# study-game-engines/directx-renderer-kurth

Hardware: AMD Instinct MI355X
Metric: physics steps/sec at 100k rigid bodies (higher is better)
Workload: dtype f32; 1 GPU; c3: 100k mixed colliders (sphere/capsule/OBB), dt 1/120 s, 30 solver iterations; bodies=100000, broadphase_pairs=611032, manifolds=251275, contacts=317267, joints=0, recoveries=0, parallelism=1 gpu

## Files before the change

### directx-renderer-kurth_amd/csrc/k_cluster_solve.hip

```cpp
#include "cluster.h"
#include "solver_rows.h"
#include "joint_solve.h"

#define CL_MAX_LOCAL_TASKS 8u
#define CLS_LANES 512u
#define CLQ_QUADS (CLS_LANES / 4u)
#define CLQ_SETS 7u
#define CLQ_REG_CONTACTS (CLQ_QUADS * CLQ_SETS)
#define CLQ_SETS_JOINTS 4u
#define CL_SPIN_LIMIT (1u << 22)

typedef u32 u32x4 __attribute__((ext_vector_type(4)));

struct QuadRow { V3 dT, aT, dN, aN; float mT, mN, bias, friction, lamN, lamT; };
#define CLQ_ZERO_FLOAT4S (2u * CLQ_QUADS + 4u)
#define CLQ_ROW_FLOAT4S 14u

struct ClLocal
{
	u32 first, count, numBodies, numShared, numColors, serialStart, numContacts, phase, key, sharedBase, numJoints;
	u32 bodyOff;
	u32 infoOff;
	u32 regContacts;
	u32 rowOff;
	u32 rowCap;
	u32 scratchBase;
	u32 colorStart[68];
};

struct ClArgs
{
	u32* counters; const ClTask* tasks; const u32* bodyList; const u32* phaseMask; const u32* sharedSlot;
	const u32* mKeySorted; const u32* mLocal; const u32* cEntry;
	const float4* rowPlanes; const float4* rowShared; float2* rowLambda; float4* rowScratch; u32 scratchContacts;
	u32 regContactsCap;
	u32 predictDiv, pollSleep;
	float4* vel; u64* flow; u64* trace;
	size_t rowCap; u32 nb, flowBytes, epoch, itBegin, itEnd, ldsFloat4s;
	const u32* jointClassStart; const uint2* taskJoints; const uint4* jointTable; float* jointUpd[MI_JOINT_TYPES]; const float4* invIw; u32 numJointClasses;
};

MI_DEV float clQuadSum(float p)
{
	float q = p + __builtin_bit_cast(float, __builtin_amdgcn_update_dpp(0, __builtin_bit_cast(int, p), 0xB1, 0xF, 0xF, false));
	return q + __builtin_bit_cast(float, __builtin_amdgcn_update_dpp(0, __builtin_bit_cast(int, q), 0x4E, 0xF, 0xF, false));
}
MI_DEV void clSolveQuad(QuadRow& r, V3& x)
{
	float vt = clQuadSum(rowDot3(x, r.dT));
	float maxFriction = r.friction * r.lamN;
	float newT = rowClampSym(__builtin_fmaf(-r.mT, vt, r.lamT), maxFriction);
	float d = newT - r.lamT; r.lamT = newT;
	x = rowFma(d, r.aT, x);
	float vn = clQuadSum(rowDot3(x, r.dN));
	float newN = fmaxf(__builtin_fmaf(-r.mN, vn - r.bias, r.lamN), 0.f);
	d = newN - r.lamN; r.lamN = newN;
	x = rowFma(d, r.aN, x);
}
// ... 18 lines not shown
template <typename PTR> MI_DEV void clStoreQuadRow(PTR P, u32 q, const QuadRow& r, u32 addr)
{
	P[3u * q] = make_float4(r.dT.x, r.dT.y, r.dT.z, r.aT.x); P[3u * q + 1u] = make_float4(r.aT.y, r.aT.z, r.dN.x, r.dN.y); P[3u * q + 2u] = make_float4(r.dN.z, r.aN.x, r.aN.y, r.aN.z);
	if (q == 0u) P[12] = make_float4(r.mT, r.mN, r.bias, r.friction);
	const u32 other = (u32)__builtin_amdgcn_update_dpp(0, (int)addr, 0xB1, 0xF, 0xF, false);
	const u32 otherPair = (u32)__builtin_amdgcn_update_dpp(0, (int)(addr | (other << 16)), 0x4E, 0xF, 0xF, false);
	if (q == 0u) P[13] = make_float4(r.lamN, r.lamT, __uint_as_float(addr | (other << 16)), __uint_as_float(otherPair));
}
MI_DEV u32 clPairAddr(u32 pair, u32 q) { return (q & 1u) ? (pair >> 16) : (pair & 0xFFFFu); }
#define CLQ_PAIR_WORD(q) (54u + ((q) >> 1))
template <typename PTR> MI_DEV void clLoadQuadRow(QuadRow& r, u32& addr, PTR P, u32 q)
{
	float4 a = P[3u * q], b = P[3u * q + 1u], c = P[3u * q + 2u], d = P[12], e = P[13];
	r.dT = v3f4(a); r.aT = v3(a.w, b.x, b.y); r.dN = v3(b.z, b.w, c.x); r.aN = v3(c.y, c.z, c.w);
	r.mT = d.x; r.mN = d.y; r.bias = d.z; r.friction = d.w; r.lamN = e.x; r.lamT = e.y;
	addr = clPairAddr(__float_as_uint(q < 2u ? e.z : e.w), q);
}

template <bool JOINTS> __global__ void __launch_bounds__(CLS_LANES) k_cl_solve(ClArgs A)
{
	extern __shared__ float4 lds[];
	__shared__ ClLocal sTask[CL_MAX_LOCAL_TASKS];
	__shared__ u32 sNumTasks, sAbort;
	const u32 tid = threadIdx.x, G = gridDim.x, quad = tid >> 2, q = tid & 3u;
	constexpr u32 SETS = JOINTS ? CLQ_SETS_JOINTS : CLQ_SETS;
	u32* status = A.counters + CTR_FLOW_STATUS;
	__amdgpu_buffer_rsrc_t rsrc = __builtin_amdgcn_make_buffer_rsrc(A.flow, 0, A.flowBytes, 0x00020000);
	const u32 zeroBase = A.ldsFloat4s - CLQ_ZERO_FLOAT4S, zeroRec = zeroBase + 2u * CLQ_QUADS, sinkRec = zeroRec + 2u;

	if (tid == 0)
	{
		if (A.trace) A.trace[(size_t)blockIdx.x * CL_TRACE_ROWS * CL_TRACE_WORDS + 15 * 32] = wall_clock64();
		u32 nT = 0, off = 0, used = 0;
		bool bad = A.counters[CTR_CL_STATUS] != 0u;
		for (u32 p = 0; p < CL_MAX_PHASES; ++p)
		{
			u32 tasksInPhase = A.counters[CTR_CL_NUM_TASKS + p];
			if (tasksInPhase > CL_TASKS_PER_PHASE * G) { bad = true; atomicOr(status, 128u); }
			off = clPhaseOffset(A.counters, p);
			u32 t = (blockIdx.x + G - (off % G)) % G;
			for (; t < tasksInPhase && !bad; t += G)
			{
				u32 key = p * CL_MAX_TASKS + t;
				const ClTask* T = A.tasks + key;
				const u32 tj = (A.jointClassStart && p == 0u) ? A.jointClassStart[(size_t)key * (CL_MAX_JOINT_CLASSES + 2u) + CL_MAX_JOINT_CLASSES] : 0u;
				if (!T->count && !tj) continue;
				if (nT == CL_MAX_LOCAL_TASKS) { bad = true; atomicOr(status, 256u); break; }
				ClLocal& L = sTask[nT];
				L.first = T->first; L.count = T->count; L.numBodies = T->numBodies; L.numShared = T->numShared; L.numColors = T->numColors; L.serialStart = T->serialStart; L.numContacts = T->numRows;
				L.phase = p; L.key = key; L.sharedBase = T->sharedBase; L.numJoints = tj;
				if (tj > CLS_LANES || (tj && nT)) { bad = true; atomicOr(status, 2048u); }
				for (u32 c = 0; c <= CL_SERIAL_COLOR + 1u; ++c) L.colorStart[c] = T->colorStart[c];
				L.colorStart[CL_SERIAL_COLOR + 2u] = L.colorStart[CL_SERIAL_COLOR + 1u]; L.colorStart[CL_SERIAL_COLOR + 3u] = L.colorStart[CL_SERIAL_COLOR + 1u];
				L.bodyOff = used; used += 2u * L.numBodies;
				L.infoOff = used * 4u; used += (3u * L.numBodies + 3u) / 4u;
				L.regContacts = (nT == 0) ? min(L.numContacts, min(CLQ_QUADS * SETS, A.regContactsCap)) : 0u;
				L.rowOff = 0; L.rowCap = 0;
				++nT;
			}
		}
		if (used + CLQ_ZERO_FLOAT4S > A.ldsFloat4s) { bad = true; atomicOr(status, 512u); }
		for (u32 k = 0; k < nT && !bad; ++k)
		{
			ClLocal& L = sTask[k];
			u32 want = L.numContacts - L.regContacts;
			u32 left = A.ldsFloat4s - used - CLQ_ZERO_FLOAT4S;
			u32 fit = left / CLQ_ROW_FLOAT4S;
			u32 cap = want < fit ? want : fit;
			L.rowOff = used; L.rowCap = cap; used += CLQ_ROW_FLOAT4S * cap; L.scratchBase = 0;
			if (want > cap) { L.scratchBase = atomicAdd(&A.counters[CTR_CL_SCRATCH], want - cap); if (L.scratchBase + (want - cap) > A.scratchContacts) { bad = true; atomicOr(status, 1024u); break; } }
		}
		if (bad) atomicOr(status, 64u);
		sNumTasks = nT; sAbort = (bad || __hip_atomic_load(status, __ATOMIC_RELAXED, __HIP_MEMORY_SCOPE_AGENT) != 0u) ? 1u : 0u;
	}
	__syncthreads();
	if (sAbort) return;
	const u32 numTasks = sNumTasks;
	if (!numTasks) return;

	for (u32 k = 0; k < numTasks; ++k)
	{
		const ClLocal& L = sTask[k];
		u32* info = (u32*)lds + L.infoOff;
		for (u32 l = tid; l < L.numBodies; l += CLS_LANES)
		{
			u32 g = A.bodyList[(size_t)L.key * CL_BODY_STRIDE + l];
			u32 pm = A.phaseMask[g];
			u32 deg = __popc(pm), rank = __popc(pm & ((1u << L.phase) - 1u));
			u32 below = pm & ((1u << L.phase) - 1u);
			u32 prev = below ? 31u - (u32)__clz(below) : 31u - (u32)__clz(pm);
			info[3 * l] = g; info[3 * l + 1] = deg | (rank << 8);
			info[3 * l + 2] = (l < L.numShared) ? A.sharedSlot[(size_t)prev * (A.nb + 1u) + g] : 0u;
			lds[L.bodyOff + 2 * l] = A.vel[2 * g]; lds[L.bodyOff + 2 * l + 1] = A.vel[2 * g + 1];
		}
	}
	for (u32 i = tid; i < CLQ_ZERO_FLOAT4S; i += CLS_LANES) lds[zeroBase + i] = make_float4(0.f, 0.f, 0.f, 0.f);
	__syncthreads();
	QuadRow rows[SETS]; u32 addr[SETS];
	{
		const ClLocal& L = sTask[0];
#pragma unroll
		for (u32 s = 0; s < SETS; ++s)
		{
			const u32 p = s * CLQ_QUADS + quad;
			rows[s].dT = rows[s].aT = rows[s].dN = rows[s].aN = v3(0.f, 0.f, 0.f); rows[s].mT = rows[s].mN = rows[s].bias = rows[s].friction = rows[s].lamN = rows[s].lamT = 0.f; addr[s] = sinkRec;
			if (p < L.regContacts) { u32 slot, kk; clBuildQuadRow(rows[s], addr[s], L, A, lds, p, q, zeroBase + 2u * quad, slot, kk); }
		}
	}
	for (u32 k = 0; k < numTasks; ++k)
	{
		const ClLocal& L = sTask[k];
		for (u32 i = quad; i < L.numContacts - L.regContacts; i += CLQ_QUADS)
		{
			QuadRow r; u32 a, slot, kk;
			clBuildQuadRow(r, a, L, A, lds, L.regContacts + i, q, zeroBase + 2u * quad, slot, kk);
			if (i < L.rowCap) clStoreQuadRow(lds + L.rowOff + i * CLQ_ROW_FLOAT4S, q, r, a);
			else clStoreQuadRow(A.rowScratch + (size_t)(L.scratchBase + i - L.rowCap) * CLQ_ROW_FLOAT4S, q, r, a);
		}
	}
	u32 tailStart0 = sTask[0].numColors, tailSet = 0, myTail = 255u;
	{
		const ClLocal& L = sTask[0];
		const u32 endPos = L.colorStart[L.numColors];
		if (L.numColors && endPos && endPos <= L.regContacts)
		{
			const u32 blk = (endPos - 1u) >> 4;
			while (tailStart0 > 0u && (L.colorStart[tailStart0 - 1u] >> 4) == blk) --tailStart0;
			if (L.numColors - tailStart0 < 2u) tailStart0 = L.numColors;
			else
			{
				tailSet = L.colorStart[tailStart0] / CLQ_QUADS;
				const u32 p = tailSet * CLQ_QUADS + quad;
				if (p >= L.colorStart[tailStart0] && p < endPos) { myTail = tailStart0; while (L.colorStart[myTail + 1u] <= p) ++myTail; }
			}
		}
		tailStart0 = __builtin_amdgcn_readfirstlane(tailStart0); tailSet = __builtin_amdgcn_readfirstlane(tailSet);
	}
	const u32 bodyOff0 = sTask[0].bodyOff;
	u32 jClass = 0xFFFFFFFFu, jType = 0, jA = 0, jB = 0, jRdA = zeroRec, jWrA = sinkRec, jRdB = zeroRec, jWrB = sinkRec; float* jRec = nullptr;
	const u32 numJoints0 = (JOINTS && sTask[0].phase == 0u) ? sTask[0].numJoints : 0u;
	if (JOINTS && tid < numJoints0)
	{
		const u32* cs = A.jointClassStart + (size_t)sTask[0].key * (CL_MAX_JOINT_CLASSES + 2u);
		uint2 e = A.taskJoints[cs[CL_MAX_JOINT_CLASSES + 1u] + tid];
		uint4 t4 = A.jointTable[e.x];
		jType = t4.x & 0xFFu; jClass = t4.x >> 8; jA = t4.z; jB = t4.w;
		jRec = A.jointUpd[jType] + (size_t)t4.y * jointUpdateFloats(jType);
		u32 la = e.y & 0xFFFFu, lb = e.y >> 16;
		if (la != CL_LOCAL_STATIC) { jRdA = bodyOff0 + 2u * la; jWrA = jRdA; }
		if (lb != CL_LOCAL_STATIC) { jRdB = bodyOff0 + 2u * lb; jWrB = jRdB; }
	}
	__syncthreads();
	u64* trace = A.trace ? A.trace + (size_t)blockIdx.x * CL_TRACE_ROWS * CL_TRACE_WORDS : nullptr;
	if (trace && tid == 0)
	{
		trace[15 * 32 + 1] = wall_clock64();
		for (u32 k = 0; k < numTasks && k < 5u; ++k) { trace[15 * 32 + 2 + 4 * k] = sTask[k].count; trace[15 * 32 + 3 + 4 * k] = sTask[k].numColors; trace[15 * 32 + 4 + 4 * k] = sTask[k].numShared; trace[15 * 32 + 5 + 4 * k] = sTask[k].phase | (sTask[k].numBodies << 8) | ((u64)sTask[k].numContacts << 32); trace[15 * 32 + 22 + k] = sTask[k].rowCap | ((u64)sTask[k].regContacts << 32); }
	}

#define CLQ_SOLVE_SET(S_, CS_, END_) if ((S_) < SETS) { const u32 pos = (S_) * CLQ_QUADS + quad; if (pos >= (CS_) && pos < (END_)) { float4 b = lds[addr[(S_) < SETS ? (S_) : 0u]]; V3 x = v3f4(b); clSolveQuad(rows[(S_) < SETS ? (S_) : 0u], x); lds[addr[(S_) < SETS ? (S_) : 0u]] = make_float4(x.x, x.y, x.z, b.w); } }
#define CLQ_PREFETCH(POS_) { const u32 in_ = max((POS_), regC) + quad - regC; if (in_ < rowCap) pfW = ((const u32*)(lds + rowOff + in_ * CLQ_ROW_FLOAT4S))[CLQ_PAIR_WORD(q)]; }
#define CLQ_SOLVE_ROWS(CS_, END_) \
	{ \
		u32 w = pfW; \
		CLQ_PREFETCH(END_) \
		for (u32 p = max((CS_), regC) + quad; p < (END_); p += CLQ_QUADS) \
		{ \
			const u32 i = p - regC; \
			QuadRow r; u32 a; float4 b; \
			float4* P = lds + rowOff + i * CLQ_ROW_FLOAT4S; \
			float4* S = A.rowScratch + (size_t)(scratchBase + i - rowCap) * CLQ_ROW_FLOAT4S; \
			u32 wn = 0u; if (p + CLQ_QUADS < (END_) && i + CLQ_QUADS < rowCap) wn = ((const u32*)(P + CLQ_QUADS * CLQ_ROW_FLOAT4S))[CLQ_PAIR_WORD(q)]; \
			if (i < rowCap) { u32 unused; a = clPairAddr(w, q); b = lds[a]; clLoadQuadRow(r, unused, P, q); } else { clLoadQuadRow(r, a, S, q); b = lds[a]; } \
			V3 x = v3f4(b); clSolveQuad(r, x); lds[a] = make_float4(x.x, x.y, x.z, b.w); \
			if (q == 0u) { if (i < rowCap) ((float2*)(P + 13))[0] = make_float2(r.lamN, r.lamT); else ((float2*)(S + 13))[0] = make_float2(r.lamN, r.lamT); } \
			w = wn; \
		} \
	}
#define CLQ_SOLVE_ROWS_LDS(CS_, END_) \
	{ \
		const u32 i = (CS_) - regC + quad, endR = (END_) - regC, w = pfW; \
		pfW = clLdsAt<u32>(lds, __umul24(min(endR + quad, lastRow), CLQ_ROW_FLOAT4S * 16u) + pairByte); \
		if (i < endR) \
		{ \
			const u32 a = clPairAddr(w, q), rowByte = __umul24(i, CLQ_ROW_FLOAT4S * 16u) + rowsByte, own = rowByte + q * 48u; \
			const float4 b = lds[a], r0 = clLdsAt<float4>(lds, own), r1 = clLdsAt<float4>(lds, own + 16u), r2 = clLdsAt<float4>(lds, own + 32u), r3 = clLdsAt<float4>(lds, rowByte + 192u); \
			const float2 lam = clLdsAt<float2>(lds, rowByte + 208u); \
			QuadRow r; r.dT = v3f4(r0); r.aT = v3(r0.w, r1.x, r1.y); r.dN = v3(r1.z, r1.w, r2.x); r.aN = v3(r2.y, r2.z, r2.w); \
			r.mT = r3.x; r.mN = r3.y; r.bias = r3.z; r.friction = r3.w; r.lamN = lam.x; r.lamT = lam.y; \
			V3 x = v3f4(b); clSolveQuad(r, x); lds[a] = make_float4(x.x, x.y, x.z, b.w); \
			if (q == 0u) *(float2*)((char*)lds + (rowByte + 208u)) = make_float2(r.lamN, r.lamT); \
		} \
	}
#define CLQ_ADVANCE(END_) \
	__syncthreads(); \
	if (stamp && c < 63u && (END_) == csNext) { trace[5 * 32 + 1 + c] = clock64(); trace[7 * 32 + c] = csNext - L.colorStart[c]; } \
	if ((END_) == csNext) { csCur = csNext; csNext = __builtin_amdgcn_readfirstlane(csAfter); ++c; } else csCur = (END_);
#define CLQ_SET_LOOP(S_) \
	if ((S_) < SETS) while (c < mainColors && csCur < min(regC, ((S_) + 1u) * CLQ_QUADS)) \
	{ \
		const u32 csAfter = L.colorStart[c + 2u];  \
		const u32 end = min(csNext, min(regC, ((S_) + 2u) * CLQ_QUADS));  \
		CLQ_SOLVE_SET(S_, csCur, end) \
		if (end > ((S_) + 1u) * CLQ_QUADS) { CLQ_SOLVE_SET((S_) + 1u, csCur, end) } \
		CLQ_ADVANCE(end) \
	}
	static_assert(CLQ_SETS <= 8u, "the colour loop below names eight sets");

	bool aborted = false;
#define CLQ_PREFETCH_TURN(K_) { const ClLocal& N = sTask[K_]; const u32 rc = N.regContacts, in_ = max(N.colorStart[0], rc) + quad - rc; if (in_ < N.rowCap) pfW = ((const u32*)(lds + N.rowOff + in_ * CLQ_ROW_FLOAT4S))[CLQ_PAIR_WORD(q)]; }
	u32 pfW = 0u;
	CLQ_PREFETCH_TURN(0u)
	u64 lastPublish = 0; u32 lastWait = 0;
	for (u32 it = A.itBegin; it < A.itEnd && !aborted; ++it)
	{
		for (u32 k = 0; k < numTasks; ++k)
		{
			const ClLocal& L = sTask[k];
			const u32* info = (const u32*)lds + L.infoOff;
			{
				if (k == 0 && lastWait > 64u && it > A.itBegin + 1u)
				{
					u64 until = lastPublish + (u64)(lastWait - lastWait / A.predictDiv);
					while (wall_clock64() < until) __builtin_amdgcn_s_sleep(8);
				}
				const u32 rel = it - A.itBegin;
				for (u32 base = 0; base < L.numShared; base += 2u * CLS_LANES)
				{
					u32 gid[2], want[2]; bool pend[2]; bool any = false;
#pragma unroll
					for (u32 qq = 0; qq < 2; ++qq)
					{
						u32 l = base + qq * CLS_LANES + tid;
// ... 40 lines not shown
			if (k == 0 && it > A.itBegin) lastWait = (u32)(wall_clock64() - lastPublish);
			if (trace && tid == 0 && it - A.itBegin < 32u && k < 5u) trace[(3 * k) * 32 + (it - A.itBegin)] = wall_clock64();
			if (JOINTS && k == 0 && numJoints0)
			{
				const u32* cs = A.jointClassStart + (size_t)L.key * (CL_MAX_JOINT_CLASSES + 2u);
				for (u32 c = 0; c < A.numJointClasses; ++c)
				{
					if (cs[c + 1u] == cs[c]) continue;
					if (jClass == c)
					{
						Vel v; float4 a0 = lds[jRdA], a1 = lds[jRdA + 1], b0 = lds[jRdB], b1 = lds[jRdB + 1];
						v.vA = v3f4(a0); v.wA = v3f4(a1); v.vB = v3f4(b0); v.wB = v3f4(b1); v.invMassA = a0.w; v.invMassB = b0.w;
						M3 IA = ldInvI(A.invIw, jA), IB = ldInvI(A.invIw, jB);
						jointSolve(jType, jRec, v, IA, IB);
						lds[jWrA] = make_float4(v.vA.x, v.vA.y, v.vA.z, v.invMassA); lds[jWrA + 1] = make_float4(v.wA.x, v.wA.y, v.wA.z, 0.f);
						lds[jWrB] = make_float4(v.vB.x, v.vB.y, v.vB.z, v.invMassB); lds[jWrB + 1] = make_float4(v.wB.x, v.wB.y, v.wB.z, 0.f);
					}
					__syncthreads();
				}
			}
			{
				const u32 numColors = __builtin_amdgcn_readfirstlane(L.numColors), serialStart = __builtin_amdgcn_readfirstlane(L.serialStart), numContacts = __builtin_amdgcn_readfirstlane(L.numContacts);
				const u32 regC = __builtin_amdgcn_readfirstlane(L.regContacts), rowOff = __builtin_amdgcn_readfirstlane(L.rowOff), rowCap = __builtin_amdgcn_readfirstlane(L.rowCap), scratchBase = __builtin_amdgcn_readfirstlane(L.scratchBase);
				const bool stamp = trace && tid == 0 && it == A.itBegin + 10u && k == 0;
				if (stamp) trace[5 * 32] = clock64();
				const u32 mainColors = (k == 0u) ? tailStart0 : numColors;
				u32 c = 0, csCur = __builtin_amdgcn_readfirstlane(L.colorStart[0]), csNext = __builtin_amdgcn_readfirstlane(L.colorStart[1]);
				CLQ_SET_LOOP(0) CLQ_SET_LOOP(1) CLQ_SET_LOOP(2) CLQ_SET_LOOP(3) CLQ_SET_LOOP(4) CLQ_SET_LOOP(5) CLQ_SET_LOOP(6) CLQ_SET_LOOP(7)
				if (rowCap >= numContacts - regC)
				{
					const u32 rowsByte = rowOff * 16u, lastRow = max(numContacts - regC, 1u) - 1u, pairByte = rowsByte + 4u * CLQ_PAIR_WORD(q);
					while (c < mainColors)
					{
						const u32 csAfter = L.colorStart[c + 2u];
						const u32 end = min(csNext, csCur + CLQ_QUADS);
						CLQ_SOLVE_ROWS_LDS(csCur, end)
						CLQ_ADVANCE(end)
					}
				}
				else while (c < mainColors)
				{
					const u32 csAfter = L.colorStart[c + 2u];
					CLQ_SOLVE_ROWS(csCur, csNext)
					CLQ_ADVANCE(csNext)
				}
				if (mainColors < numColors)
				{
#define CLQ_TAIL(S_) case S_: if ((S_) < SETS && myTail != 255u) for (u32 ct = mainColors; ct < numColors; ++ct) { if (myTail == ct) { float4 b = lds[addr[(S_) < SETS ? (S_) : 0u]]; V3 x = v3f4(b); clSolveQuad(rows[(S_) < SETS ? (S_) : 0u], x); lds[addr[(S_) < SETS ? (S_) : 0u]] = make_float4(x.x, x.y, x.z, b.w); } __builtin_amdgcn_fence(__ATOMIC_ACQ_REL, "wavefront"); } break;
					switch (tailSet) { CLQ_TAIL(0) CLQ_TAIL(1) CLQ_TAIL(2) CLQ_TAIL(3) CLQ_TAIL(4) CLQ_TAIL(5) CLQ_TAIL(6) CLQ_TAIL(7) default: break; }
#undef CLQ_TAIL
					__syncthreads();
					if (stamp) for (u32 ct = mainColors; ct < numColors && ct < 63u; ++ct) { trace[5 * 32 + 1 + ct] = clock64(); trace[7 * 32 + ct] = L.colorStart[ct + 1u] - L.colorStart[ct]; }
				}
				if (serialStart < numContacts) CLQ_PREFETCH(serialStart)
				for (u32 sp = serialStart; sp < numContacts; ++sp)
				{
					if (sp < regC)
					{
						switch (sp / CLQ_QUADS)
						{
							case 0: CLQ_SOLVE_SET(0u, sp, sp + 1u) break; case 1: CLQ_SOLVE_SET(1u, sp, sp + 1u) break; case 2: CLQ_SOLVE_SET(2u, sp, sp + 1u) break; case 3: CLQ_SOLVE_SET(3u, sp, sp + 1u) break;
							case 4: CLQ_SOLVE_SET(4u, sp, sp + 1u) break; case 5: CLQ_SOLVE_SET(5u, sp, sp + 1u) break; case 6: CLQ_SOLVE_SET(6u, sp, sp + 1u) break; default: CLQ_SOLVE_SET(7u, sp, sp + 1u) break;
						}
					}
					else { CLQ_SOLVE_ROWS(sp, sp + 1u) }
					__syncthreads();
				}
			}
			if (trace && tid == 0 && it - A.itBegin < 32u && k < 5u) trace[(3 * k + 1) * 32 + (it - A.itBegin)] = wall_clock64();
			for (u32 l = tid; l < L.numShared; l += CLS_LANES)
			{
				u32 g = info[3 * l], ti = info[3 * l + 1];
				u32 deg = ti & 0xFFu, rank = ti >> 8;
				u32 want = A.epoch + (it - A.itBegin) * deg + rank;
				u32 rec = (L.sharedBase + l) * 32u;
				float4 b0 = lds[L.bodyOff + 2 * l], b1 = lds[L.bodyOff + 2 * l + 1];
				if (it + 1u == A.itEnd && rank + 1u == deg) { A.vel[2 * g] = b0; A.vel[2 * g + 1] = make_float4(b1.x, b1.y, b1.z, 0.f); }
				else
				{
					u32x4 h1 = { __float_as_uint(b1.x), __float_as_uint(b1.y), __float_as_uint(b1.z), want + 1u };
					u32x4 h0 = { __float_as_uint(b0.x), __float_as_uint(b0.y), __float_as_uint(b0.z), want + 1u };
					__builtin_amdgcn_raw_buffer_store_b128(h1, rsrc, rec + 16u, 0, 16);
					__builtin_amdgcn_raw_buffer_store_b128(h0, rsrc, rec, 0, 16);
				}
			}
// ... 1 lines not shown
			CLQ_PREFETCH_TURN(k + 1u < numTasks ? k + 1u : 0u)
		}
	}
	if (aborted) return;

	for (u32 k = 0; k < numTasks; ++k)
	{
		const ClLocal& L = sTask[k];
		const u32* info = (const u32*)lds + L.infoOff;
		for (u32 l = L.numShared + tid; l < L.numBodies; l += CLS_LANES)
		{
			u32 g = info[3 * l];
			float4 b1 = lds[L.bodyOff + 2 * l + 1];
			A.vel[2 * g] = lds[L.bodyOff + 2 * l]; A.vel[2 * g + 1] = make_float4(b1.x, b1.y, b1.z, 0.f);
		}
		if (q == 0u)
		{
			if (k == 0)
			{
#pragma unroll
				for (u32 s = 0; s < SETS; ++s)
				{
					const u32 p = s * CLQ_QUADS + quad;
					if (p < L.regContacts) { const u32 e = A.cEntry[(size_t)4u * L.first + p]; A.rowLambda[(size_t)(e >> 12) * A.rowCap + L.first + (e & 0xFFFu)] = make_float2(rows[s].lamN, rows[s].lamT); }
				}
			}
			for (u32 i = quad; i < L.numContacts - L.regContacts; i += CLQ_QUADS)
			{
				const u32 e = A.cEntry[(size_t)4u * L.first + L.regContacts + i];
				const float4 lam = i < L.rowCap ? lds[L.rowOff + i * CLQ_ROW_FLOAT4S + 13u] : A.rowScratch[(size_t)(L.scratchBase + i - L.rowCap) * CLQ_ROW_FLOAT4S + 13u];
				A.rowLambda[(size_t)(e >> 12) * A.rowCap + L.first + (e & 0xFFFu)] = make_float2(lam.x, lam.y);
			}
		}
	}
#undef CLQ_SET_LOOP
#undef CLQ_ADVANCE
#undef CLQ_SOLVE_ROWS
#undef CLQ_SOLVE_ROWS_LDS
#undef CLQ_PREFETCH
#undef CLQ_PREFETCH_TURN
#undef CLQ_SOLVE_SET
}

bool cluster_solves_joints(const World& w) { return w.cluster.jointsInCluster && w.cluster.jointsEnabled; }

u32 cluster_solve_setup(const World& w)
{
	int maxLds = 0;
	MI_CHECK(hipDeviceGetAttribute(&maxLds, hipDeviceAttributeMaxSharedMemoryPerBlock, w.device));
	hipFuncAttributes fa = {};
	MI_CHECK(hipFuncGetAttributes(&fa, (const void*)k_cl_solve<true>));
	size_t dyn = (maxLds > 0 ? (size_t)maxLds : 65536) - fa.sharedSizeBytes - 256;
	dyn &= ~(size_t)15;
// ... 24 lines not shown

void launch_cluster_solve(World& w, u32 itBegin, u32 itEnd)
{
	if (itBegin >= itEnd) return;
	size_t words = (size_t)(w.nb + 1) * CL_MAX_PHASES * 4;
	if (w.cluster.flow.cap < words) { w.cluster.flow.ensure(words, w.stream); w.cluster.flowEpoch = 0; if (w.lastError) return; }
	if (w.cluster.flowEpoch == 0 || w.cluster.flowEpoch >= 0xFFFEu)
	{
		MI_CHECK(hipMemsetAsync(w.cluster.flow.p, 0, sizeof(u64) * words, w.stream));
		w.cluster.flowEpoch = 0;
	}
	w.cluster.flowEpoch++;
	if (w.cluster.flowTestAbortStep == w.stats.numInternalSteps)
	{
		u32 one = 16u;
		MI_CHECK(hipMemcpyAsync(w.dCounters.p + CTR_FLOW_STATUS, &one, sizeof(u32), hipMemcpyHostToDevice, w.stream));
		MI_CHECK(hipStreamSynchronize(w.stream));
	}
	const size_t scratchContacts = std::min<size_t>(2 * w.pairCap, 512u * 1024u);
	w.cluster.rowScratch.ensure(scratchContacts * CLQ_ROW_FLOAT4S, w.stream);
	if (w.lastError) return;
	if (itBegin) MI_CHECK(hipMemsetAsync(w.dCounters.p + CTR_CL_SCRATCH, 0, sizeof(u32), w.stream));
	ClArgs A;
	A.rowScratch = w.cluster.rowScratch.p; A.scratchContacts = (u32)scratchContacts; A.regContactsCap = w.cluster.regContactsCap;
	A.counters = w.dCounters.p; A.tasks = (const ClTask*)w.cluster.tasks.p; A.bodyList = w.cluster.bodyList.p; A.phaseMask = w.cluster.phaseMask.p; A.sharedSlot = w.cluster.sharedSlot.p;
	A.mKeySorted = w.mKeySorted.p; A.mLocal = w.cluster.local.p; A.cEntry = w.cluster.entry.p;
	A.rowPlanes = w.rowPlanes.p; A.rowShared = w.rowShared.p; A.rowLambda = w.rowLambda.p; A.vel = w.vel.p; A.flow = w.cluster.flow.p; A.trace = w.cluster.flowTrace.p; A.predictDiv = CL_PREDICT_DIV; A.pollSleep = CL_POLL_SLEEP;
	A.rowCap = w.rowCap; A.nb = w.nb; A.flowBytes = (u32)(words * sizeof(u64)); A.epoch = w.cluster.flowEpoch << 16; A.itBegin = itBegin; A.itEnd = itEnd;
	A.ldsFloat4s = w.cluster.ldsBytes / 16u;
	const bool withJoints = cluster_solves_joints(w);
	A.jointClassStart = withJoints ? w.cluster.jointClassStart.p : nullptr; A.taskJoints = w.cluster.taskJoints.p; A.jointTable = w.cluster.jointTable.p; A.invIw = w.invIw.p; A.numJointClasses = withJoints ? w.cluster.numJointClasses : 0u;
	for (u32 t = 0; t < MI_JOINT_TYPES; ++t) A.jointUpd[t] = w.joints[t].dUpdate.p;
	if (withJoints) hipLaunchKernelGGL(k_cl_solve<true>, dim3(w.cluster.blocks), dim3(CLS_LANES), w.cluster.ldsBytes, w.stream, A);
	else hipLaunchKernelGGL(k_cl_solve<false>, dim3(w.cluster.blocks), dim3(CLS_LANES), w.cluster.ldsBytes, w.stream, A);
}
```

### directx-renderer-kurth_amd/csrc/world.h

```cpp
#pragma once
#include "mi_common.h"
#include "../../include/mi_physics.h"
#include <vector>
#include <string>
#include <algorithm>
#include <type_traits>

struct mi_distance_constraint { float localAnchorA[3], localAnchorB[3], globalLength; };
struct mi_ball_constraint { float localAnchorA[3], localAnchorB[3]; };
struct mi_fixed_constraint { float initialInvRotationDifference[4], localAnchorA[3], localAnchorB[3]; };
struct mi_hinge_constraint
{
	float localAnchorA[3], localAnchorB[3], localHingeAxisA[3], localHingeAxisB[3];
	float minRotationLimit, maxRotationLimit, maxMotorTorque; u32 motorType; float motorVelocity;
	float localHingeTangentA[3], localHingeBitangentA[3], localHingeTangentB[3];
};
struct mi_cone_twist_constraint
{
	float localAnchorA[3], localAnchorB[3], localLimitAxisA[3], localLimitAxisB[3];
	float localLimitTangentA[3], localLimitBitangentA[3], localLimitTangentB[3];
	float swingLimit, twistLimit; u32 swingMotorType; float swingMotorVelocity, maxSwingMotorTorque, swingMotorAxis;
	u32 twistMotorType; float twistMotorVelocity, maxTwistMotorTorque;
};
struct mi_slider_constraint
// ... 193 lines not shown
	{
		std::vector<HCloth> cloths;
		bool dirty = true, stateOnDevice = false;
		u32 iterations[3] = { 0, 1, 0 };
		DevBuf<float> planes; u32 stride = 0;
		DevBuf<uint2> ab; DevBuf<float2> restIms; DevBuf<float4> temp; DevBuf<uint8_t> descs; DevBuf<u32> list;
		u32 numSmall = 0, maxSmallParticles = 0;
	} cloth;
	void uploadCloths(); void downloadCloths();

	struct Slab
	{
		DevBuf<uint8_t> code; DevBuf<u32> fresh; u32 rank = 0, size = 0, axis = 0, stamp = 0; float lo = 0.f, hi = 0.f, margin = 0.f;
	} slab;

	struct Cluster
	{
		bool enabled = true;
		bool jointsEnabled = true;
		u32 blocksLimit = 0, failStreak = 0, taskWeight = 64u * 1000u, taskWeightLater = 64u * 500u;
		u32 taskWeightComp = 64u * 200u;
		u32 ldsBytes = 0, blocks = 0, cooldown = 0;
		u32 regContactsCap = ~0u;
		bool compIdle = false;

		bool sortDue = true; u32 sortAge = 0, sortBodies = 0;
		DevBuf<u32> keys, keysSorted, vals, sorted, rank, wsum, cum, taskKey, taskPos, taskCount;
		DevBuf<u32> jointBodyMask; bool jointListsValid = false;
		DevBuf<u32> compLabel, leftList;
		DevBuf<u32> chunk; u32 chunkJointVersion = ~0u; bool chunkWithJoints = false;
		DevBuf<u32> rep, jointTask, jointPos, jointCount; u32 numJoints = 0;

		DevBuf<u32> phaseMask, pre, local, entry, taskStart, bodyList, sharedSlot;
		DevBuf<uint8_t> tasks;
		DevBuf<float4> rowScratch;
		DevBuf<u32> jointStart, jointList; DevBuf<uint4> jointTable; DevBuf<uint2> taskJoints; DevBuf<u32> jointClassStart;
		u32 numJointClasses = 0; bool jointsInCluster = false;
		DevBuf<u64> flow;
		DevBuf<u64> flowTrace;
		u32 flowEpoch = 0;
		DevBuf<float4> velBackup; u32 flowTestAbortStep = ~0u;
	} cluster;
	void recoverFlow(); int resolvePendingFlow();

	struct Zones
	{
// ... 106 lines not shown
```

### directx-renderer-kurth_amd/csrc/world.hip

```cpp
#include "world.h"
#include <cstdio>
#include <cstring>
#include <atomic>

thread_local std::string g_createError;
thread_local World* g_currentWorld = nullptr;

void mi_set_error(hipError_t e, const char* file, int line)
{
	char buf[512];
	snprintf(buf, sizeof(buf), "HIP error %d (%s) at %s:%d", (int)e, hipGetErrorString(e), file, line);
	if (g_currentWorld) { if (!g_currentWorld->lastError) { g_currentWorld->lastError = MI_ERR_HIP; g_currentWorld->lastErrorText = buf; } }
	else g_createError = buf;
}

template <typename T> void DevBuf<T>::ensure(size_t n, hipStream_t s, bool keep)
{
	if (n <= cap) return;
	size_t newCap = std::max(n, cap + cap / 2);
	T* np = nullptr;
	MI_CHECK(hipMalloc((void**)&np, newCap * sizeof(T)));
	if (!np) return;
	if (keep && p && cap) { MI_CHECK(hipMemcpyAsync(np, p, cap * sizeof(T), hipMemcpyDeviceToDevice, s)); MI_CHECK(hipStreamSynchronize(s)); }
	if (p) MI_CHECK(hipFree(p));
// ... 11 lines not shown
	if (const char* e = getenv("MI_NARROW_SIDE_STREAM")) narrowSideStream = atoi(e) != 0;
	if (narrowSideStream)
	{
		MI_CHECK(hipStreamCreateWithFlags(&narrowStream, hipStreamNonBlocking));
		MI_CHECK(hipEventCreateWithFlags(&narrowFork, hipEventDisableTiming | hipEventDisableSystemFence));
		MI_CHECK(hipEventCreateWithFlags(&narrowJoin, hipEventDisableTiming | hipEventDisableSystemFence));
		if (!narrowStream || !narrowFork || !narrowJoin) narrowSideStream = false;
	}
	MI_CHECK(hipHostMalloc((void**)&hCounters, CTR_WORDS * sizeof(u32), hipHostMallocDefault));
	if (hCounters) memset(hCounters, 0, CTR_WORDS * sizeof(u32));
	dCounters.ensure(CTR_WORDS, stream);
	if (dCounters.p) MI_CHECK(hipMemsetAsync(dCounters.p, 0, CTR_WORDS * sizeof(u32), stream));
	timing.stageEvents.resize(STAGE_RING * 6);
	for (auto& e : timing.stageEvents) MI_CHECK(hipEventCreateWithFlags(&e, hipEventDisableSystemFence));
	MI_CHECK(hipEventCreateWithFlags(&countersEvent, hipEventDisableTiming));
	validate = getenv("MI_PHYSICS_VALIDATE") != nullptr;
	cluster.enabled = getenv("MI_PHYSICS_NO_CLUSTER") == nullptr;
	cluster.jointsEnabled = getenv("MI_CLUSTER_NO_JOINTS") == nullptr;
	if (const char* e = getenv("MI_FLOW_TEST_ABORT")) cluster.flowTestAbortStep = (u32)atoi(e);
	if (const char* e = getenv("MI_CLUSTER_TASK")) { cluster.taskWeight = 64u * (u32)std::max(16, atoi(e)); cluster.taskWeightLater = std::min(cluster.taskWeight, cluster.taskWeightLater); cluster.taskWeightComp = std::min(cluster.taskWeight, cluster.taskWeightComp); }
	if (getenv("MI_PHYSICS_REPLAY")) replay.referenceOrder = true;
	if (const char* e = getenv("MI_CLUSTER_BLOCKS")) cluster.blocksLimit = (u32)std::max(1, atoi(e));
	if (const char* e = getenv("MI_CLUSTER_REG_CONTACTS")) cluster.regContactsCap = (u32)std::max(0, atoi(e));
	if (const char* e = getenv("MI_CLUSTER_TASK_LATER")) cluster.taskWeightLater = 64u * (u32)std::max(16, atoi(e));
	if (const char* e = getenv("MI_CLUSTER_TASK_COMP")) cluster.taskWeightComp = 64u * (u32)std::min(1 << 20, std::max(16, atoi(e)));
	if (dCounters.p)
	{
		u32 box[6] = { 0xFFFFFFFFu, 0xFFFFFFFFu, 0xFFFFFFFFu, 0u, 0u, 0u };
		MI_CHECK(hipMemcpyAsync(dCounters.p + CTR_CL_BBOX, box, sizeof(box), hipMemcpyHostToDevice, stream));
		MI_CHECK(hipStreamSynchronize(stream));
	}
}

World::~World()
{
	g_currentWorld = this;
	if (narrowStream) (void)hipStreamSynchronize(narrowStream);
	if (stream) (void)hipStreamSynchronize(stream);
	for (auto& e : timing.stageEvents) if (e) (void)hipEventDestroy(e);
	if (countersEvent) (void)hipEventDestroy(countersEvent);
	if (hCounters) (void)hipHostFree(hCounters);
	if (narrowFork) (void)hipEventDestroy(narrowFork);
	if (narrowJoin) (void)hipEventDestroy(narrowJoin);
	if (narrowStream) (void)hipStreamDestroy(narrowStream);
	if (stream) (void)hipStreamDestroy(stream);
	g_currentWorld = nullptr;
// ... 376 lines not shown
```

Measured before the change: 579.1 steps/s.

## Reorder contact placement: spill rows first, LDS rows next, register rows last

Rearranges where each cluster task's contact rows live in the solve order. Rows spilled to global scratch now come first, LDS-resident rows follow, and register-held quads take the tail of the contact range instead of the head. Colour iteration becomes three phases (scratch, LDS fast path, register sets), with register colour starts rebased in a shared array. The aim is to keep the fast LDS-only loop even when some rows spill, and to let the register tail line up with the final colours. It also adds an MI_CLUSTER_LDS_ROWS cap for experiments, at the cost of more complex indexing and new edge cases at colour boundaries.

```diff
diff --git a/directx-renderer-kurth_amd/csrc/k_cluster_solve.hip b/directx-renderer-kurth_amd/csrc/k_cluster_solve.hip
--- a/directx-renderer-kurth_amd/csrc/k_cluster_solve.hip
+++ b/directx-renderer-kurth_amd/csrc/k_cluster_solve.hip
@@ -21,10 +21,8 @@
 	u32 first, count, numBodies, numShared, numColors, serialStart, numContacts, phase, key, sharedBase, numJoints;
 	u32 bodyOff;
 	u32 infoOff;
-	u32 regContacts;
-	u32 rowOff;
-	u32 rowCap;
-	u32 scratchBase;
+	u32 regContacts, spill, rowOff, rowCap, scratchBase;
+	u32 ldsColors;
 	u32 colorStart[68];
 };
 
@@ -34,6 +32,7 @@
 	const u32* mKeySorted; const u32* mLocal; const u32* cEntry;
 	const float4* rowPlanes; const float4* rowShared; float2* rowLambda; float4* rowScratch; u32 scratchContacts;
 	u32 regContactsCap;
+	u32 ldsRowsCap;
 	u32 predictDiv, pollSleep;
 	float4* vel; u64* flow; u64* trace;
 	size_t rowCap; u32 nb, flowBytes, epoch, itBegin, itEnd, ldsFloat4s;
@@ -98,6 +97,7 @@
 	extern __shared__ float4 lds[];
 	__shared__ ClLocal sTask[CL_MAX_LOCAL_TASKS];
 	__shared__ u32 sNumTasks, sAbort;
+	__shared__ u32 sRegStart[CL_SERIAL_COLOR + 4u];
 	const u32 tid = threadIdx.x, G = gridDim.x, quad = tid >> 2, q = tid & 3u;
 	constexpr u32 SETS = JOINTS ? CLQ_SETS_JOINTS : CLQ_SETS;
 	u32* status = A.counters + CTR_FLOW_STATUS;
@@ -131,19 +131,23 @@
 				L.bodyOff = used; used += 2u * L.numBodies;
 				L.infoOff = used * 4u; used += (3u * L.numBodies + 3u) / 4u;
 				L.regContacts = (nT == 0) ? min(L.numContacts, min(CLQ_QUADS * SETS, A.regContactsCap)) : 0u;
-				L.rowOff = 0; L.rowCap = 0;
+				L.rowOff = 0; L.rowCap = 0; L.spill = 0;
+				const u32 regBase = L.numContacts - L.regContacts;
+				L.ldsColors = 0; while (L.ldsColors < L.numColors && L.colorStart[L.ldsColors + 1u] <= regBase) ++L.ldsColors;
+				if (nT == 0) for (u32 c = 0; c < CL_SERIAL_COLOR + 4u; ++c) sRegStart[c] = L.colorStart[c] - regBase;
 				++nT;
 			}
 		}
 		if (used + CLQ_ZERO_FLOAT4S > A.ldsFloat4s) { bad = true; atomicOr(status, 512u); }
+		u32 ldsRowsLeft = A.ldsRowsCap;
 		for (u32 k = 0; k < nT && !bad; ++k)
 		{
 			ClLocal& L = sTask[k];
 			u32 want = L.numContacts - L.regContacts;
 			u32 left = A.ldsFloat4s - used - CLQ_ZERO_FLOAT4S;
-			u32 fit = left / CLQ_ROW_FLOAT4S;
+			u32 fit = min(left / CLQ_ROW_FLOAT4S, ldsRowsLeft);
 			u32 cap = want < fit ? want : fit;
-			L.rowOff = used; L.rowCap = cap; used += CLQ_ROW_FLOAT4S * cap; L.scratchBase = 0;
+			L.rowOff = used; L.rowCap = cap; used += CLQ_ROW_FLOAT4S * cap; ldsRowsLeft -= cap; L.scratchBase = 0; L.spill = want - cap;
 			if (want > cap) { L.scratchBase = atomicAdd(&A.counters[CTR_CL_SCRATCH], want - cap); if (L.scratchBase + (want - cap) > A.scratchContacts) { bad = true; atomicOr(status, 1024u); break; } }
 		}
 		if (bad) atomicOr(status, 64u);
@@ -175,38 +179,39 @@
 	QuadRow rows[SETS]; u32 addr[SETS];
 	{
 		const ClLocal& L = sTask[0];
+		const u32 regBase = L.numContacts - L.regContacts;
 #pragma unroll
 		for (u32 s = 0; s < SETS; ++s)
 		{
 			const u32 p = s * CLQ_QUADS + quad;
 			rows[s].dT = rows[s].aT = rows[s].dN = rows[s].aN = v3(0.f, 0.f, 0.f); rows[s].mT = rows[s].mN = rows[s].bias = rows[s].friction = rows[s].lamN = rows[s].lamT = 0.f; addr[s] = sinkRec;
-			if (p < L.regContacts) { u32 slot, kk; clBuildQuadRow(rows[s], addr[s], L, A, lds, p, q, zeroBase + 2u * quad, slot, kk); }
+			if (p < L.regContacts) { u32 slot, kk; clBuildQuadRow(rows[s], addr[s], L, A, lds, regBase + p, q, zeroBase + 2u * quad, slot, kk); }
 		}
 	}
 	for (u32 k = 0; k < numTasks; ++k)
 	{
 		const ClLocal& L = sTask[k];
-		for (u32 i = quad; i < L.numContacts - L.regContacts; i += CLQ_QUADS)
+		for (u32 p = quad; p < L.numContacts - L.regContacts; p += CLQ_QUADS)
 		{
 			QuadRow r; u32 a, slot, kk;
-			clBuildQuadRow(r, a, L, A, lds, L.regContacts + i, q, zeroBase + 2u * quad, slot, kk);
-			if (i < L.rowCap) clStoreQuadRow(lds + L.rowOff + i * CLQ_ROW_FLOAT4S, q, r, a);
-			else clStoreQuadRow(A.rowScratch + (size_t)(L.scratchBase + i - L.rowCap) * CLQ_ROW_FLOAT4S, q, r, a);
+			clBuildQuadRow(r, a, L, A, lds, p, q, zeroBase + 2u * quad, slot, kk);
+			if (p >= L.spill) clStoreQuadRow(lds + L.rowOff + (p - L.spill) * CLQ_ROW_FLOAT4S, q, r, a);
+			else clStoreQuadRow(A.rowScratch + (size_t)(L.scratchBase + p) * CLQ_ROW_FLOAT4S, q, r, a);
 		}
 	}
 	u32 tailStart0 = sTask[0].numColors, tailSet = 0, myTail = 255u;
 	{
 		const ClLocal& L = sTask[0];
-		const u32 endPos = L.colorStart[L.numColors];
-		if (L.numColors && endPos && endPos <= L.regContacts)
-		{
-			const u32 blk = (endPos - 1u) >> 4;
-			while (tailStart0 > 0u && (L.colorStart[tailStart0 - 1u] >> 4) == blk) --tailStart0;
+		const u32 regBase = L.numContacts - L.regContacts, endPos = L.colorStart[L.numColors];
+		if (L.numColors && endPos > regBase)
+		{
+			const u32 blk = (endPos - regBase - 1u) >> 4;
+			while (tailStart0 > 0u && L.colorStart[tailStart0 - 1u] >= regBase && ((L.colorStart[tailStart0 - 1u] - regBase) >> 4) == blk) --tailStart0;
 			if (L.numColors - tailStart0 < 2u) tailStart0 = L.numColors;
 			else
 			{
-				tailSet = L.colorStart[tailStart0] / CLQ_QUADS;
-				const u32 p = tailSet * CLQ_QUADS + quad;
+				tailSet = (L.colorStart[tailStart0] - regBase) / CLQ_QUADS;
+				const u32 p = regBase + tailSet * CLQ_QUADS + quad;
 				if (p >= L.colorStart[tailStart0] && p < endPos) { myTail = tailStart0; while (L.colorStart[myTail + 1u] <= p) ++myTail; }
 			}
 		}
@@ -231,31 +236,31 @@
 	if (trace && tid == 0)
 	{
 		trace[15 * 32 + 1] = wall_clock64();
-		for (u32 k = 0; k < numTasks && k < 5u; ++k) { trace[15 * 32 + 2 + 4 * k] = sTask[k].count; trace[15 * 32 + 3 + 4 * k] = sTask[k].numColors; trace[15 * 32 + 4 + 4 * k] = sTask[k].numShared; trace[15 * 32 + 5 + 4 * k] = sTask[k].phase | (sTask[k].numBodies << 8) | ((u64)sTask[k].numContacts << 32); trace[15 * 32 + 22 + k] = sTask[k].rowCap | ((u64)sTask[k].regContacts << 32); }
+		for (u32 k = 0; k < numTasks && k < 5u; ++k) { trace[15 * 32 + 2 + 4 * k] = sTask[k].count; trace[15 * 32 + 3 + 4 * k] = sTask[k].numColors; trace[15 * 32 + 4 + 4 * k] = sTask[k].numShared; trace[15 * 32 + 5 + 4 * k] = sTask[k].phase | (sTask[k].numBodies << 8) | ((u64)sTask[k].numContacts << 32); trace[15 * 32 + 22 + k] = sTask[k].rowCap | ((u64)sTask[k].regContacts << 32); trace[15 * 32 + 27 + k] = sTask[k].spill | ((u64)(k == 0u ? sTask[0].numColors - tailStart0 : 0u) << 32); }
 	}
 
 #define CLQ_SOLVE_SET(S_, CS_, END_) if ((S_) < SETS) { const u32 pos = (S_) * CLQ_QUADS + quad; if (pos >= (CS_) && pos < (END_)) { float4 b = lds[addr[(S_) < SETS ? (S_) : 0u]]; V3 x = v3f4(b); clSolveQuad(rows[(S_) < SETS ? (S_) : 0u], x); lds[addr[(S_) < SETS ? (S_) : 0u]] = make_float4(x.x, x.y, x.z, b.w); } }
-#define CLQ_PREFETCH(POS_) { const u32 in_ = max((POS_), regC) + quad - regC; if (in_ < rowCap) pfW = ((const u32*)(lds + rowOff + in_ * CLQ_ROW_FLOAT4S))[CLQ_PAIR_WORD(q)]; }
+#define CLQ_PREFETCH(POS_) { const u32 in_ = max((POS_), spill) + quad - spill; if (in_ < rowCap) pfW = ((const u32*)(lds + rowOff + in_ * CLQ_ROW_FLOAT4S))[CLQ_PAIR_WORD(q)]; }
 #define CLQ_SOLVE_ROWS(CS_, END_) \
 	{ \
 		u32 w = pfW; \
 		CLQ_PREFETCH(END_) \
-		for (u32 p = max((CS_), regC) + quad; p < (END_); p += CLQ_QUADS) \
+		for (u32 p = (CS_) + quad; p < (END_); p += CLQ_QUADS) \
 		{ \
-			const u32 i = p - regC; \
+			const bool inLds = p >= spill; \
 			QuadRow r; u32 a; float4 b; \
-			float4* P = lds + rowOff + i * CLQ_ROW_FLOAT4S; \
-			float4* S = A.rowScratch + (size_t)(scratchBase + i - rowCap) * CLQ_ROW_FLOAT4S; \
-			u32 wn = 0u; if (p + CLQ_QUADS < (END_) && i + CLQ_QUADS < rowCap) wn = ((const u32*)(P + CLQ_QUADS * CLQ_ROW_FLOAT4S))[CLQ_PAIR_WORD(q)]; \
-			if (i < rowCap) { u32 unused; a = clPairAddr(w, q); b = lds[a]; clLoadQuadRow(r, unused, P, q); } else { clLoadQuadRow(r, a, S, q); b = lds[a]; } \
+			float4* P = lds + rowOff + (inLds ? p - spill : 0u) * CLQ_ROW_FLOAT4S; \
+			float4* S = A.rowScratch + (size_t)(scratchBase + (inLds ? 0u : p)) * CLQ_ROW_FLOAT4S; \
+			u32 wn = 0u; if (p + CLQ_QUADS < (END_) && p + CLQ_QUADS >= spill) wn = ((const u32*)(lds + rowOff + (p + CLQ_QUADS - spill) * CLQ_ROW_FLOAT4S))[CLQ_PAIR_WORD(q)]; \
+			if (inLds) { u32 unused; a = clPairAddr(w, q); b = lds[a]; clLoadQuadRow(r, unused, P, q); } else { clLoadQuadRow(r, a, S, q); b = lds[a]; } \
 			V3 x = v3f4(b); clSolveQuad(r, x); lds[a] = make_float4(x.x, x.y, x.z, b.w); \
-			if (q == 0u) { if (i < rowCap) ((float2*)(P + 13))[0] = make_float2(r.lamN, r.lamT); else ((float2*)(S + 13))[0] = make_float2(r.lamN, r.lamT); } \
+			if (q == 0u) { if (inLds) ((float2*)(P + 13))[0] = make_float2(r.lamN, r.lamT); else ((float2*)(S + 13))[0] = make_float2(r.lamN, r.lamT); } \
 			w = wn; \
 		} \
 	}
 #define CLQ_SOLVE_ROWS_LDS(CS_, END_) \
 	{ \
-		const u32 i = (CS_) - regC + quad, endR = (END_) - regC, w = pfW; \
+		const u32 i = (CS_) - spill + quad, endR = (END_) - spill, w = pfW; \
 		pfW = clLdsAt<u32>(lds, __umul24(min(endR + quad, lastRow), CLQ_ROW_FLOAT4S * 16u) + pairByte); \
 		if (i < endR) \
 		{ \
@@ -270,12 +275,12 @@
 	}
 #define CLQ_ADVANCE(END_) \
 	__syncthreads(); \
-	if (stamp && c < 63u && (END_) == csNext) { trace[5 * 32 + 1 + c] = clock64(); trace[7 * 32 + c] = csNext - L.colorStart[c]; } \
+	if (stamp && c < 63u && (END_) == csNext) { trace[5 * 32 + 1 + c] = clock64(); trace[7 * 32 + c] = L.colorStart[c + 1u] - L.colorStart[c]; } \
 	if ((END_) == csNext) { csCur = csNext; csNext = __builtin_amdgcn_readfirstlane(csAfter); ++c; } else csCur = (END_);
 #define CLQ_SET_LOOP(S_) \
 	if ((S_) < SETS) while (c < mainColors && csCur < min(regC, ((S_) + 1u) * CLQ_QUADS)) \
 	{ \
-		const u32 csAfter = L.colorStart[c + 2u];  \
+		const u32 csAfter = sRegStart[c + 2u];  \
 		const u32 end = min(csNext, min(regC, ((S_) + 2u) * CLQ_QUADS));  \
 		CLQ_SOLVE_SET(S_, csCur, end) \
 		if (end > ((S_) + 1u) * CLQ_QUADS) { CLQ_SOLVE_SET((S_) + 1u, csCur, end) } \
@@ -284,7 +289,7 @@
 	static_assert(CLQ_SETS <= 8u, "the colour loop below names eight sets");
 
 	bool aborted = false;
-#define CLQ_PREFETCH_TURN(K_) { const ClLocal& N = sTask[K_]; const u32 rc = N.regContacts, in_ = max(N.colorStart[0], rc) + quad - rc; if (in_ < N.rowCap) pfW = ((const u32*)(lds + N.rowOff + in_ * CLQ_ROW_FLOAT4S))[CLQ_PAIR_WORD(q)]; }
+#define CLQ_PREFETCH_TURN(K_) { const ClLocal& N = sTask[K_]; const u32 sp_ = N.spill, in_ = max(N.colorStart[0], sp_) + quad - sp_; if (in_ < N.rowCap) pfW = ((const u32*)(lds + N.rowOff + in_ * CLQ_ROW_FLOAT4S))[CLQ_PAIR_WORD(q)]; }
 	u32 pfW = 0u;
 	CLQ_PREFETCH_TURN(0u)
 	u64 lastPublish = 0; u32 lastWait = 0;
@@ -371,28 +376,40 @@
 			{
 				const u32 numColors = __builtin_amdgcn_readfirstlane(L.numColors), serialStart = __builtin_amdgcn_readfirstlane(L.serialStart), numContacts = __builtin_amdgcn_readfirstlane(L.numContacts);
 				const u32 regC = __builtin_amdgcn_readfirstlane(L.regContacts), rowOff = __builtin_amdgcn_readfirstlane(L.rowOff), rowCap = __builtin_amdgcn_readfirstlane(L.rowCap), scratchBase = __builtin_amdgcn_readfirstlane(L.scratchBase);
+				const u32 spill = __builtin_amdgcn_readfirstlane(L.spill), ldsColors = __builtin_amdgcn_readfirstlane(L.ldsColors), regBase = numContacts - regC;
 				const bool stamp = trace && tid == 0 && it == A.itBegin + 10u && k == 0;
 				if (stamp) trace[5 * 32] = clock64();
 				const u32 mainColors = (k == 0u) ? tailStart0 : numColors;
 				u32 c = 0, csCur = __builtin_amdgcn_readfirstlane(L.colorStart[0]), csNext = __builtin_amdgcn_readfirstlane(L.colorStart[1]);
-				CLQ_SET_LOOP(0) CLQ_SET_LOOP(1) CLQ_SET_LOOP(2) CLQ_SET_LOOP(3) CLQ_SET_LOOP(4) CLQ_SET_LOOP(5) CLQ_SET_LOOP(6) CLQ_SET_LOOP(7)
-				if (rowCap >= numContacts - regC)
-				{
-					const u32 rowsByte = rowOff * 16u, lastRow = max(numContacts - regC, 1u) - 1u, pairByte = rowsByte + 4u * CLQ_PAIR_WORD(q);
-					while (c < mainColors)
+				if (__builtin_expect(regBase != 0u, 0))
+				{
+					while (c < mainColors && csCur < spill)
 					{
 						const u32 csAfter = L.colorStart[c + 2u];
-						const u32 end = min(csNext, csCur + CLQ_QUADS);
-						CLQ_SOLVE_ROWS_LDS(csCur, end)
+						const u32 end = min(csNext, spill);
+						CLQ_SOLVE_ROWS(csCur, end)
 						CLQ_ADVANCE(end)
 					}
-				}
-				else while (c < mainColors)
-				{
-					const u32 csAfter = L.colorStart[c + 2u];
-					CLQ_SOLVE_ROWS(csCur, csNext)
-					CLQ_ADVANCE(csNext)
-				}
+					{
+						const u32 rowsByte = rowOff * 16u, lastRow = max(rowCap, 1u) - 1u, pairByte = rowsByte + 4u * CLQ_PAIR_WORD(q);
+						while (c < ldsColors)
+						{
+							const u32 csAfter = L.colorStart[c + 2u];
+							const u32 end = min(csNext, csCur + CLQ_QUADS);
+							CLQ_SOLVE_ROWS_LDS(csCur, end)
+							CLQ_ADVANCE(end)
+						}
+						while (c < mainColors && csCur < regBase)
+						{
+							const u32 csAfter = L.colorStart[c + 2u];
+							const u32 end = min(regBase, csCur + CLQ_QUADS);
+							CLQ_SOLVE_ROWS_LDS(csCur, end)
+							CLQ_ADVANCE(end)
+						}
+					}
+					csCur -= regBase; csNext -= regBase;
+				}
+				CLQ_SET_LOOP(0) CLQ_SET_LOOP(1) CLQ_SET_LOOP(2) CLQ_SET_LOOP(3) CLQ_SET_LOOP(4) CLQ_SET_LOOP(5) CLQ_SET_LOOP(6) CLQ_SET_LOOP(7)
 				if (mainColors < numColors)
 				{
 #define CLQ_TAIL(S_) case S_: if ((S_) < SETS && myTail != 255u) for (u32 ct = mainColors; ct < numColors; ++ct) { if (myTail == ct) { float4 b = lds[addr[(S_) < SETS ? (S_) : 0u]]; V3 x = v3f4(b); clSolveQuad(rows[(S_) < SETS ? (S_) : 0u], x); lds[addr[(S_) < SETS ? (S_) : 0u]] = make_float4(x.x, x.y, x.z, b.w); } __builtin_amdgcn_fence(__ATOMIC_ACQ_REL, "wavefront"); } break;
@@ -404,12 +421,13 @@
 				if (serialStart < numContacts) CLQ_PREFETCH(serialStart)
 				for (u32 sp = serialStart; sp < numContacts; ++sp)
 				{
-					if (sp < regC)
+					if (sp >= regBase)
 					{
-						switch (sp / CLQ_QUADS)
+						const u32 rp = sp - regBase;
+						switch (rp / CLQ_QUADS)
 						{
-							case 0: CLQ_SOLVE_SET(0u, sp, sp + 1u) break; case 1: CLQ_SOLVE_SET(1u, sp, sp + 1u) break; case 2: CLQ_SOLVE_SET(2u, sp, sp + 1u) break; case 3: CLQ_SOLVE_SET(3u, sp, sp + 1u) break;
-							case 4: CLQ_SOLVE_SET(4u, sp, sp + 1u) break; case 5: CLQ_SOLVE_SET(5u, sp, sp + 1u) break; case 6: CLQ_SOLVE_SET(6u, sp, sp + 1u) break; default: CLQ_SOLVE_SET(7u, sp, sp + 1u) break;
+							case 0: CLQ_SOLVE_SET(0u, rp, rp + 1u) break; case 1: CLQ_SOLVE_SET(1u, rp, rp + 1u) break; case 2: CLQ_SOLVE_SET(2u, rp, rp + 1u) break; case 3: CLQ_SOLVE_SET(3u, rp, rp + 1u) break;
+							case 4: CLQ_SOLVE_SET(4u, rp, rp + 1u) break; case 5: CLQ_SOLVE_SET(5u, rp, rp + 1u) break; case 6: CLQ_SOLVE_SET(6u, rp, rp + 1u) break; default: CLQ_SOLVE_SET(7u, rp, rp + 1u) break;
 						}
 					}
 					else { CLQ_SOLVE_ROWS(sp, sp + 1u) }
@@ -457,13 +475,13 @@
 				for (u32 s = 0; s < SETS; ++s)
 				{
 					const u32 p = s * CLQ_QUADS + quad;
-					if (p < L.regContacts) { const u32 e = A.cEntry[(size_t)4u * L.first + p]; A.rowLambda[(size_t)(e >> 12) * A.rowCap + L.first + (e & 0xFFFu)] = make_float2(rows[s].lamN, rows[s].lamT); }
-				}
-			}
-			for (u32 i = quad; i < L.numContacts - L.regContacts; i += CLQ_QUADS)
-			{
-				const u32 e = A.cEntry[(size_t)4u * L.first + L.regContacts + i];
-				const float4 lam = i < L.rowCap ? lds[L.rowOff + i * CLQ_ROW_FLOAT4S + 13u] : A.rowScratch[(size_t)(L.scratchBase + i - L.rowCap) * CLQ_ROW_FLOAT4S + 13u];
+					if (p < L.regContacts) { const u32 e = A.cEntry[(size_t)4u * L.first + (L.numContacts - L.regContacts) + p]; A.rowLambda[(size_t)(e >> 12) * A.rowCap + L.first + (e & 0xFFFu)] = make_float2(rows[s].lamN, rows[s].lamT); }
+				}
+			}
+			for (u32 p = quad; p < L.numContacts - L.regContacts; p += CLQ_QUADS)
+			{
+				const u32 e = A.cEntry[(size_t)4u * L.first + p];
+				const float4 lam = p >= L.spill ? lds[L.rowOff + (p - L.spill) * CLQ_ROW_FLOAT4S + 13u] : A.rowScratch[(size_t)(L.scratchBase + p) * CLQ_ROW_FLOAT4S + 13u];
 				A.rowLambda[(size_t)(e >> 12) * A.rowCap + L.first + (e & 0xFFFu)] = make_float2(lam.x, lam.y);
 			}
 		}
@@ -534,7 +552,7 @@
 	if (w.lastError) return;
 	if (itBegin) MI_CHECK(hipMemsetAsync(w.dCounters.p + CTR_CL_SCRATCH, 0, sizeof(u32), w.stream));
 	ClArgs A;
-	A.rowScratch = w.cluster.rowScratch.p; A.scratchContacts = (u32)scratchContacts; A.regContactsCap = w.cluster.regContactsCap;
+	A.rowScratch = w.cluster.rowScratch.p; A.scratchContacts = (u32)scratchContacts; A.regContactsCap = w.cluster.regContactsCap; A.ldsRowsCap = w.cluster.ldsRowsCap;
 	A.counters = w.dCounters.p; A.tasks = (const ClTask*)w.cluster.tasks.p; A.bodyList = w.cluster.bodyList.p; A.phaseMask = w.cluster.phaseMask.p; A.sharedSlot = w.cluster.sharedSlot.p;
 	A.mKeySorted = w.mKeySorted.p; A.mLocal = w.cluster.local.p; A.cEntry = w.cluster.entry.p;
 	A.rowPlanes = w.rowPlanes.p; A.rowShared = w.rowShared.p; A.rowLambda = w.rowLambda.p; A.vel = w.vel.p; A.flow = w.cluster.flow.p; A.trace = w.cluster.flowTrace.p; A.predictDiv = CL_PREDICT_DIV; A.pollSleep = CL_POLL_SLEEP;
diff --git a/directx-renderer-kurth_amd/csrc/world.h b/directx-renderer-kurth_amd/csrc/world.h
--- a/directx-renderer-kurth_amd/csrc/world.h
+++ b/directx-renderer-kurth_amd/csrc/world.h
@@ -239,6 +239,7 @@
 		u32 taskWeightComp = 64u * 200u;
 		u32 ldsBytes = 0, blocks = 0, cooldown = 0;
 		u32 regContactsCap = ~0u;
+		u32 ldsRowsCap = ~0u;
 		bool compIdle = false;
 
 		bool sortDue = true; u32 sortAge = 0, sortBodies = 0;
diff --git a/directx-renderer-kurth_amd/csrc/world.hip b/directx-renderer-kurth_amd/csrc/world.hip
--- a/directx-renderer-kurth_amd/csrc/world.hip
+++ b/directx-renderer-kurth_amd/csrc/world.hip
@@ -57,6 +57,7 @@
 	if (getenv("MI_PHYSICS_REPLAY")) replay.referenceOrder = true;
 	if (const char* e = getenv("MI_CLUSTER_BLOCKS")) cluster.blocksLimit = (u32)std::max(1, atoi(e));
 	if (const char* e = getenv("MI_CLUSTER_REG_CONTACTS")) cluster.regContactsCap = (u32)std::max(0, atoi(e));
+	if (const char* e = getenv("MI_CLUSTER_LDS_ROWS")) cluster.ldsRowsCap = (u32)std::max(0, atoi(e));
 	if (const char* e = getenv("MI_CLUSTER_TASK_LATER")) cluster.taskWeightLater = 64u * (u32)std::max(16, atoi(e));
 	if (const char* e = getenv("MI_CLUSTER_TASK_COMP")) cluster.taskWeightComp = 64u * (u32)std::min(1 << 20, std::max(16, atoi(e)));
 	if (dCounters.p)
```

Measured after the change: 618.9 steps/s (median of 6 runs). 6.9% higher.
